# tudelft-iv/instance_stixels

Hardware: NVIDIA B200
Metric: stixel frames/sec @1024x2048 (higher is better)
Workload: dtype f32

## Files before the change

### instance_stixels_b200/csrc/context.cu

```cuda
#include <algorithm>
#include <cstdio>
#include <cstdlib>
#include <cstring>
#include <map>
#include <mutex>
#include <string>
#include <vector>

#include "host_model.h"
#include "kernels.h"

namespace isx {

static thread_local std::string g_last_error;
constexpr int kStageSlots = 8;
constexpr int kRoadSlots = 4;
constexpr int kResultSets = 4;
constexpr int kProfEvents = 9;
constexpr int kTraceStamps = 11;

static int fail(isx_context *ctx, int code, const std::string &msg);

struct RoadKey {
  int vhor;
  float tilt, height, alpha;
  bool operator<(const RoadKey &o) const {
    if (vhor != o.vhor) return vhor < o.vhor;
    if (tilt != o.tilt) return tilt < o.tilt;
    if (height != o.height) return height < o.height;
    return alpha < o.alpha;
  }
};

}

struct isx_context {
  int device = 0;
  bool configured_parts[8] = {false, false, false, false, false, false, false, false};
  bool initialized = false;
  isx::HostModel model;
  isx::KParams kp{};
  int max_batch = 0, chunk = 0;
  int chunk_unary = 0;
  int last_launch_frames = 0;
  std::string last_error;

  cudaStream_t s_tables = nullptr, s_compute = nullptr, s_emit = nullptr, s_h2d = nullptr, s_d2h = nullptr;
  cudaEvent_t ev_dp_done[2] = {nullptr, nullptr}, ev_emit_done[2] = {nullptr, nullptr};
  cudaEvent_t ev_tab_done[2] = {nullptr, nullptr};
  cudaEvent_t ev_user = nullptr;
  cudaEvent_t ev_in_ready[2] = {nullptr, nullptr}, ev_in_free[2] = {nullptr, nullptr};
  cudaEvent_t ev_chunk_done = nullptr;
  uint16_t *d_in_disp16[2] = {nullptr, nullptr};
  int16_t *d_in_seg16[2] = {nullptr, nullptr};

  std::vector<void *> allocations;
  float *d_in_disp[2] = {nullptr, nullptr};
  int32_t *d_in_seg[2] = {nullptr, nullptr};
  float *d_single_disp = nullptr;
  int32_t *d_single_seg = nullptr;
  isx::BatchBuffers buf;
  struct ChunkSet {
    float *stat = nullptr;
    uint32_t *records_b = nullptr;
    float4 *dp = nullptr;
    float *pm = nullptr;
    int *err = nullptr;
    float *joined = nullptr;
    float *object_lut = nullptr;
    int *col_flags = nullptr;
  } sets[2];
  int last_set = 0;
  struct RoadSlot {
    float *ground = nullptr;
    int *vhor = nullptr;
    cudaEvent_t ev_free = nullptr;
  } roads[isx::kRoadSlots];
  unsigned long long road_next = 0;
  int last_road_slot = 0;
  bool overlap_tables = true;
  bool emit_join_pending = false;
  struct ResultSet {
    bool allocated = false;
    isx_section *d_sections = nullptr;
    int *d_nsections = nullptr;
    isx_instance *d_inst = nullptr;
    int *d_inst_count = nullptr;
    int *d_cursors = nullptr;
    isx_section *h_sections = nullptr, *m_sections = nullptr;
    isx_instance *h_inst = nullptr, *m_inst = nullptr;
    int *h_counts = nullptr, *m_counts = nullptr;
    isx_packed_frame *h_frames = nullptr, *m_frames = nullptr;
    int sections_cap = 0, inst_cap = 0;
  } rs[isx::kResultSets];
  int cur = 0;
  int *d_raster_table = nullptr;
  int *d_export_col = nullptr;
  int inst_cap = 0;
  float *d_export_cost = nullptr;
  int *d_export_index = nullptr;

  float *h_ground = nullptr;
  int *h_vhor = nullptr;
  cudaEvent_t ev_stage_done[8] = {nullptr, nullptr, nullptr, nullptr, nullptr, nullptr, nullptr, nullptr};
  unsigned long long stage_next = 0;
  cudaEvent_t ev_batch_done[isx::kResultSets] = {};
  int batch_n[isx::kResultSets] = {};
  int batch_set[isx::kResultSets] = {};
  isx_section *batch_sections[isx::kResultSets] = {};
  bool batch_direct[isx::kResultSets] = {};
  isx_section *direct_sections = nullptr;
  bool results_stay_on_device = false;
  int last_waited_set = -1;
  unsigned long long submitted = 0, waited = 0;
  unsigned long long dp_units_pairwise = 0;
  unsigned long long dp_units_total = 0;
  int host_slot = 0;

  std::map<isx::RoadKey, std::vector<float>> road_cache;
  std::mutex road_cache_mutex;
  isx_road *h_stage_roads = nullptr;
  isx_road *d_batch_roads = nullptr;
  bool last_roads_device = false;
  isx_road single_road{0, 0.f, 0.f, 0.f};
  bool single_has_road = false;
  int last_batch = 0;
  int last_chunk_first = 0;
  int last_chunk_n = 0;
  bool last_pairwise = false;
  std::vector<isx_road> last_roads;
// ... 133 lines not shown
  ISX_TRY(c, cudaEventRecord(c->ev_stage_done[stage], st));
  return rslot;
}

static int stage_road_tables(isx_context *c, const isx_road *roads, int n, cudaStream_t st) {
  const int H = c->kp.rows;
  const int stage = (int)(c->stage_next++ % kStageSlots);
  ISX_TRY(c, cudaEventSynchronize(c->ev_stage_done[stage]));
  float *hg = c->h_ground + (size_t)stage * c->chunk * 3 * H;
  int *hv = c->h_vhor + (size_t)stage * c->chunk;
  for (int i = 0; i < n; i++) {
    copy_road_tables(c, roads[i], hg + (size_t)i * 3 * H);
    hv[i] = H - roads[i].vhor - 1;
  }
  return send_road_tables(c, stage, n, st);
}

struct StageFill {
  isx_context *c;
  int stage, n;
};

static void CUDART_CB fill_stage_from_roads(void *arg) {
  const StageFill p = *static_cast<StageFill *>(arg);
  delete static_cast<StageFill *>(arg);
  isx_context *c = p.c;
  const int H = c->kp.rows;
  const isx_road *roads = c->h_stage_roads + (size_t)p.stage * c->chunk;
  float *hg = c->h_ground + (size_t)p.stage * c->chunk * 3 * H;
  int *hv = c->h_vhor + (size_t)p.stage * c->chunk;
  for (int i = 0; i < p.n; i++) {
    copy_road_tables(c, roads[i], hg + (size_t)i * 3 * H);
    hv[i] = H - roads[i].vhor - 1;
  }
}

static int stage_device_road_tables(isx_context *c, const isx_road *d_roads, int n, cudaStream_t st) {
  const int stage = (int)(c->stage_next++ % kStageSlots);
  ISX_TRY(c, cudaStreamWaitEvent(st, c->ev_stage_done[stage], 0));
  ISX_TRY(c, cudaMemcpyAsync(c->h_stage_roads + (size_t)stage * c->chunk, d_roads, sizeof(isx_road) * n,
                             cudaMemcpyDeviceToHost, st));
  ISX_TRY(c, cudaLaunchHostFunc(st, fill_stage_from_roads, new StageFill{c, stage, n}));
  return send_road_tables(c, stage, n, st);
}

static int enqueue_chunk(isx_context *c, bool pairwise, int first, int n, const float *d_disp,
                         const int32_t *d_seg, const isx_road *roads, int slot, int road_slot = -1) {
  const KParams &kp = c->kp;
  const int H = kp.rows, C = kp.realcols;
  const isx_context::ChunkSet &cs = c->sets[slot];
  cudaStream_t st = c->s_tables, s = c->s_compute, se = c->s_emit;
  ISX_TRY(c, cudaStreamWaitEvent(st, c->ev_emit_done[slot], 0));
  if (!c->overlap_tables) ISX_TRY(c, cudaStreamWaitEvent(st, c->ev_dp_done[slot ^ 1], 0));
  if (road_slot < 0) {
    road_slot = stage_road_tables(c, roads, n, st);
    if (road_slot < 0) return road_slot;
  }
  const isx_context::RoadSlot &rd = c->roads[road_slot];
  ISX_TRY(c, cudaMemsetAsync(cs.err, 0, sizeof(int) * n, st));
  isx_context::ResultSet &R = c->rs[c->cur];
  BatchBuffers b = c->buf;
  b.ground = rd.ground; b.vhor = rd.vhor; b.stat = cs.stat;
  b.records_b = cs.records_b; b.dp = cs.dp; b.pm = cs.pm;
  b.joined = cs.joined; b.object_lut = cs.object_lut; b.col_flags = cs.col_flags;
  b.error_flag = cs.err;
  b.disparity = d_disp;
  b.segmentation = d_seg;
  b.sections = R.d_sections + (size_t)first * C * kMaxSections;
  b.n_sections = R.d_nsections + (size_t)first * C;
  auto mark = [&](cudaStream_t st) {
    if (!c->profiling) return;
    if (c->prof_used >= c->prof_events.size()) {
      cudaEvent_t e;
      cudaEventCreate(&e);
      c->prof_events.push_back(e);
    }
    cudaEventRecord(c->prof_events[c->prof_used++], st);
  };
  mark(st);
  launch_join_columns(kp, b, n, st);
  mark(st);
  if (pairwise) launch_frame_tables(kp, b, n, st);
  mark(st);
  launch_column_tables(kp, b, n, st);
  mark(st);
  ISX_TRY(c, cudaEventRecord(c->ev_tab_done[slot], st));
  ISX_TRY(c, cudaStreamWaitEvent(s, c->ev_tab_done[slot], 0));
  mark(s);
  launch_dp(kp, b, n, pairwise, s);
  {
    const unsigned long long nt = (unsigned long long)(H + 31) / 32;
    c->dp_units_total += (unsigned long long)n * C * (nt * (nt + 1) / 2);
    const char *ex = std::getenv("ISX_UNARY_EXHAUSTIVE");
    const bool walks_all = (pairwise && !pairwise_walk_used(n * C, b.qrows != nullptr)) || (!pairwise && ex && std::atoi(ex) != 0);
    c->dp_units_pairwise += walks_all ? (unsigned long long)n * C * (nt * (nt + 1) / 2) : 0;
  }
  mark(s);
  ISX_TRY(c, cudaEventRecord(c->ev_dp_done[slot], s));
  ISX_TRY(c, cudaStreamWaitEvent(se, c->ev_dp_done[slot], 0));
  mark(se);
  launch_emit(kp, b, n, pairwise, se);
  mark(se);
  launch_grouping(kp, b, n, se);
  {
    PackArgs a;
    a.sections = b.sections; a.n_sections = b.n_sections;
    a.cand_count = b.cand_count; a.cand_idx = b.cand_idx; a.cand_label = b.cand_label;
    a.err = cs.err; a.col_offset = b.pack_offset;
    a.inst_out = R.d_inst + (size_t)first * c->inst_cap; a.inst_count_out = R.d_inst_count + first;
    a.inst_cap = c->inst_cap; a.cursors = R.d_cursors;
    a.h_padded = c->direct_sections ? c->direct_sections + (size_t)first * C * kMaxSections : nullptr;
    a.h_sections = R.m_sections; a.h_sections_cap = c->results_stay_on_device ? 0 : R.sections_cap;
    a.h_inst = R.m_inst; a.h_inst_cap = c->results_stay_on_device ? 0 : R.inst_cap;
    a.h_counts = R.m_counts + (size_t)first * C; a.h_frames = R.m_frames + first;
    launch_pack(kp, a, n, se);
  }
  mark(se);
  ISX_TRY(c, cudaEventRecord(c->ev_emit_done[slot], se));
  ISX_TRY(c, cudaEventRecord(rd.ev_free, se));
  ISX_TRY(c, cudaGetLastError());
  c->last_chunk_first = first;
  c->last_chunk_n = n;
  c->last_pairwise = pairwise;
  c->last_set = slot;
  c->last_road_slot = road_slot;
  return ISX_OK;
}

static isx_section *device_view_of(isx_section *sections) {
  if (!sections) return nullptr;
  if (const char *e = std::getenv("ISX_NO_DIRECT"))
    if (std::atoi(e) != 0) return nullptr;
  cudaPointerAttributes attr;
  if (cudaPointerGetAttributes(&attr, sections) != cudaSuccess) {
    cudaGetLastError();
    return nullptr;
  }
  if (attr.type != cudaMemoryTypeHost || !attr.devicePointer) return nullptr;
  return static_cast<isx_section *>(attr.devicePointer);
}

static int begin_batch(isx_context *c) {
  ISX_TRY(c, cudaMemsetAsync(c->rs[c->cur].d_cursors, 0, 2 * sizeof(int), c->s_emit));
  return ISX_OK;
}

static int alloc_result_set(isx_context *c, int i) {
  isx_context::ResultSet &R = c->rs[i];
  if (R.allocated) return ISX_OK;
  const size_t C = c->kp.realcols, MB = c->max_batch;
  ISX_TRY(c, dev_alloc(c, &R.d_sections, MB * C * kMaxSections));
  ISX_TRY(c, cudaMemset(R.d_sections, 0, MB * C * kMaxSections * sizeof(isx_section)));
  ISX_TRY(c, dev_alloc(c, &R.d_nsections, MB * C));
  ISX_TRY(c, dev_alloc(c, &R.d_inst, MB * (size_t)c->inst_cap));
  ISX_TRY(c, dev_alloc(c, &R.d_inst_count, MB));
  ISX_TRY(c, dev_alloc(c, &R.d_cursors, 2));
  ISX_TRY(c, cudaMemset(R.d_cursors, 0, 2 * sizeof(int)));
  size_t budget = 100;
  if (c->kp.rows > kShortRows) budget = ((size_t)c->kp.rows * 100 + kShortRows - 1) / kShortRows;
  if (const char *e = std::getenv("ISX_PACK_BUDGET")) budget = std::atoi(e) > 0 ? (size_t)std::atoi(e) : budget;
  budget = budget < (size_t)kMaxSections ? budget : (size_t)kMaxSections;
  R.sections_cap = R.inst_cap = (int)(MB * C * budget);
  const unsigned flags = cudaHostAllocMapped | cudaHostAllocPortable;
  ISX_TRY(c, cudaHostAlloc(&R.h_sections, sizeof(isx_section) * (size_t)R.sections_cap, flags));
  ISX_TRY(c, cudaHostAlloc(&R.h_inst, sizeof(isx_instance) * (size_t)R.inst_cap, flags));
  ISX_TRY(c, cudaHostAlloc(&R.h_counts, sizeof(int) * MB * C, flags));
  ISX_TRY(c, cudaHostAlloc(&R.h_frames, sizeof(isx_packed_frame) * MB, flags));
// ... 108 lines not shown
  m.prior_weight = prior_weight; m.disparity_weight = disparity_weight; m.segmentation_weight = segmentation_weight;
  m.instance_weight = 0.0;
  if (segmentation_weight > 1e-5) {
    m.instance_weight = instance_weight / segmentation_weight;
    if (instance_weight < 1e-8) m.instance_weight = 0.0;
  }
  return ISX_OK;
}
int isx_set_probabilities(isx_handle h, float pout, float pout_sky, float pground_given_nexist,
                          float pobject_given_nexist, float psky_given_nexist, float pnexist_dis, float pground,
                          float pobject, float psky, float pord, float pgrav, float pblg) {
  if (!h) return fail(h, ISX_ERR_INVALID_ARGUMENT, "null handle");
  HostModel &m = h->model;
  m.pout = pout; m.pout_sky = pout_sky;
  m.pnexists_given_ground = (pground_given_nexist * pnexist_dis) / pground;
  m.pnexists_given_object = (pobject_given_nexist * pnexist_dis) / pobject;
  m.pnexists_given_sky = (psky_given_nexist * pnexist_dis) / psky;
  m.pord = pord; m.pgrav = pgrav; m.pblg = pblg;
  return ISX_OK;
}
int isx_set_camera_parameters(isx_handle h, float focal, float baseline, float sigma_camera_tilt,
                              float sigma_camera_height, float camera_center_x, float camera_center_y) {
  if (!h) return fail(h, ISX_ERR_INVALID_ARGUMENT, "null handle");
  HostModel &m = h->model;
  m.focal = focal; m.baseline = baseline;
  m.sigma_camera_tilt = sigma_camera_tilt * (3.1416f) / 180.0f;
  m.sigma_camera_height = sigma_camera_height;
  m.camera_center_x = camera_center_x; m.camera_center_y = camera_center_y;
  return ISX_OK;
}
int isx_set_model_parameters(isx_handle h, int column_step, int median_join, float epsilon, float range_objects_z,
                             int width_margin) {
  if (!h) return fail(h, ISX_ERR_INVALID_ARGUMENT, "null handle");
  HostModel &m = h->model;
  m.column_step = column_step; m.median_join = median_join != 0; m.epsilon = epsilon;
  m.range_objects_z = range_objects_z; m.width_margin = width_margin;
  return ISX_OK;
}

int isx_initialize(isx_handle h, int max_batch) {
  if (!h) return fail(h, ISX_ERR_INVALID_ARGUMENT, "null handle");
  if (h->initialized) return fail(h, ISX_ERR_INVALID_ARGUMENT, "already initialized: call Finish() first");
  if (max_batch < 1) return fail(h, ISX_ERR_INVALID_ARGUMENT, "max_batch must be >= 1");
  HostModel &m = h->model;
  if (m.rows <= 0 || m.cols <= 0 || m.max_dis <= 0 || m.column_step <= 0)
    return fail(h, ISX_ERR_INVALID_ARGUMENT, "configuration is not set");
  if (m.rows > ISX_MAX_ROWS) return fail(h, ISX_ERR_UNSUPPORTED, "rows > ISX_MAX_ROWS (2047) is not supported");
  if (m.max_dis > 256) return fail(h, ISX_ERR_UNSUPPORTED, "max_dis > 256 is not supported");
  if (m.n_classes != 19 || m.n_channels != 21)
    return fail(h, ISX_ERR_UNSUPPORTED, "the Cityscapes layout (19 classes + 2 offsets) is hard-wired like Cityscapes.h");
  if (m.column_step > 16) return fail(h, ISX_ERR_UNSUPPORTED, "column_step > 16 is not supported");
  ISX_TRY(h, cudaSetDevice(h->device));
  m.derive();
  fill_kparams(h);
  const KParams &kp = h->kp;
  const size_t H = kp.rows, W = kp.cols, C = kp.realcols, D = kp.max_dis;
  if (C == 0) return fail(h, ISX_ERR_INVALID_ARGUMENT, "no stixel columns");
  h->max_batch = max_batch;
  int chunk = 64, chunk_unary = 32;
  if (m.rows > kShortRows) {
    const size_t budget = 64 * chunk_frame_bytes(kShortRows, 2048, kRecStride, 2048 / 4, m.max_dis);
    const size_t per_frame = chunk_frame_bytes(m.rows, m.cols, rec_stride_for_rows(m.rows), m.realcols, m.max_dis);
    const size_t fit = budget / per_frame;
    chunk = fit < 1 ? 1 : fit < 64 ? (int)fit : 64;
    chunk_unary = chunk < 32 ? chunk : 32;
  }
  if (const char *e = std::getenv("ISX_CHUNK")) chunk = chunk_unary = std::atoi(e) > 0 ? std::atoi(e) : chunk;
  h->chunk = chunk < max_batch ? chunk : max_batch;
  h->chunk_unary = chunk_unary < h->chunk ? chunk_unary : h->chunk;
  h->last_launch_frames = h->chunk_unary;
  h->kp.lut_cols = h->chunk * (int)C;
  const size_t ch = h->chunk, MB = max_batch;
  const size_t cap = C * kMaxSections;
  h->inst_cap = (int)cap;

  {
    int prio_lo = 0, prio_hi = 0;
    ISX_TRY(h, cudaDeviceGetStreamPriorityRange(&prio_lo, &prio_hi));
    int prio_mid = prio_lo;
    if (const char *e = std::getenv("ISX_TABLES_PRIO"))
      prio_mid = (std::atoi(e) != 0 && prio_hi < prio_lo - 1) ? prio_hi + 1 : prio_lo;
    ISX_TRY(h, cudaStreamCreateWithPriority(&h->s_compute, cudaStreamNonBlocking, prio_lo));
    ISX_TRY(h, cudaStreamCreateWithPriority(&h->s_tables, cudaStreamNonBlocking, prio_mid));
    ISX_TRY(h, cudaStreamCreateWithPriority(&h->s_emit, cudaStreamNonBlocking, prio_hi));
  }
  ISX_TRY(h, cudaStreamCreateWithFlags(&h->s_h2d, cudaStreamNonBlocking));
  ISX_TRY(h, cudaStreamCreateWithFlags(&h->s_d2h, cudaStreamNonBlocking));
  for (int i = 0; i < 2; i++) {
    ISX_TRY(h, cudaEventCreateWithFlags(&h->ev_in_ready[i], cudaEventDisableTiming));
    ISX_TRY(h, cudaEventCreateWithFlags(&h->ev_in_free[i], cudaEventDisableTiming));
    ISX_TRY(h, cudaEventCreateWithFlags(&h->ev_dp_done[i], cudaEventDisableTiming));
    ISX_TRY(h, cudaEventCreateWithFlags(&h->ev_emit_done[i], cudaEventDisableTiming));
    ISX_TRY(h, cudaEventCreateWithFlags(&h->ev_tab_done[i], cudaEventDisableTiming));
  }
  ISX_TRY(h, cudaEventCreateWithFlags(&h->ev_chunk_done, cudaEventDisableTiming));
  ISX_TRY(h, cudaEventCreateWithFlags(&h->ev_user, cudaEventDisableTiming));

  BatchBuffers &b = h->buf;
  for (int i = 0; i < kRoadSlots; i++) {
    ISX_TRY(h, dev_alloc(h, &h->roads[i].ground, ch * 3 * H));
    ISX_TRY(h, dev_alloc(h, &h->roads[i].vhor, ch));
    ISX_TRY(h, cudaEventCreateWithFlags(&h->roads[i].ev_free, cudaEventDisableTiming));
  }
  h->road_next = 0;
  for (int i = 0; i < 2; i++) {
    ISX_TRY(h, dev_alloc(h, &h->d_in_disp[i], ch * H * W));
    ISX_TRY(h, dev_alloc(h, &h->d_in_seg[i], ch * seg_elems(h)));
    ISX_TRY(h, cudaMemset(h->d_in_seg[i], 0, ch * seg_elems(h) * sizeof(int32_t)));
  }
  ISX_TRY(h, dev_alloc(h, &h->d_single_disp, H * W));
  ISX_TRY(h, dev_alloc(h, &h->d_single_seg, seg_elems(h)));
  for (int i = 0; i < 2; i++) {
    isx_context::ChunkSet &cs = h->sets[i];
    ISX_TRY(h, dev_alloc(h, &cs.stat, ch * H * kStatWords));
    ISX_TRY(h, dev_alloc(h, &cs.records_b, ch * C * kRecBWords * (size_t)kp.rec_stride));
    ISX_TRY(h, cudaMemset(cs.records_b, 0, ch * C * kRecBWords * (size_t)kp.rec_stride * sizeof(uint32_t)));
    ISX_TRY(h, dev_alloc(h, &cs.pm, ch * C * H));
    ISX_TRY(h, cudaMemset(cs.pm, 0, ch * C * H * sizeof(float)));
    ISX_TRY(h, dev_alloc(h, &cs.dp, ch * C * H));
    ISX_TRY(h, dev_alloc(h, &cs.err, ch));
    ISX_TRY(h, dev_alloc(h, &cs.joined, ch * C * H));
    ISX_TRY(h, dev_alloc(h, &cs.object_lut, lut_buffer_bytes(ch * C, D * (size_t)kp.lut_stride * 4) / 4));
    ISX_TRY(h, dev_alloc(h, &cs.col_flags, ch * C));
    ISX_TRY(h, cudaMemset(cs.col_flags, 0, ch * C * sizeof(int)));
  }
  ISX_TRY(h, dev_alloc(h, &b.cand_count, ch * kInstanceClasses));
  ISX_TRY(h, dev_alloc(h, &b.cand_offset, ch * (C + 1) * kInstanceClasses));
  ISX_TRY(h, dev_alloc(h, &b.cand_xy, ch * kInstanceClasses * cap));
  ISX_TRY(h, dev_alloc(h, &b.cand_idx, ch * kInstanceClasses * cap));
  ISX_TRY(h, dev_alloc(h, &b.cand_core, ch * kInstanceClasses * cap));
  ISX_TRY(h, dev_alloc(h, &b.cand_label, ch * kInstanceClasses * cap));
  ISX_TRY(h, dev_alloc(h, &b.cand_scratch, ch * kInstanceClasses * cap));
  ISX_TRY(h, dev_alloc(h, &b.pack_offset, ch * (C + 1)));
  ISX_TRY(h, dev_alloc(h, &b.dp_units, 1));
  if (pairwise_walk_enabled()) {
    ISX_TRY(h, dev_alloc(h, &b.qrows, ch * C * (size_t)kp.rec_stride * kDynWords));
    ISX_TRY(h, cudaMemset(b.qrows, 0, ch * C * (size_t)kp.rec_stride * kDynWords * sizeof(float)));
  }
  ISX_TRY(h, cudaMemset(b.dp_units, 0, sizeof(unsigned long long)));
  h->cur = 0;
  if (int rc = alloc_result_set(h, 0)) return rc;
  ISX_TRY(h, dev_alloc(h, &h->d_raster_table, MB * C * kMaxSections));
  ISX_TRY(h, dev_alloc(h, &h->d_export_col, MB * C));
  ISX_TRY(h, dev_alloc(h, &h->d_export_cost, C * H * 3));
  ISX_TRY(h, dev_alloc(h, &h->d_export_index, C * H * 3));

  float *d_tmp = nullptr;
  ISX_TRY(h, dev_alloc(h, &d_tmp, D * D));
  ISX_TRY(h, cudaMemcpy(d_tmp, m.obj_cost_lut.data(), sizeof(float) * D * D, cudaMemcpyHostToDevice));
  b.obj_cost_lut = d_tmp;
  {
    const size_t Dp = (D + 31) & ~(size_t)31;
    std::vector<float> t(D * Dp, 0.0f);
    for (size_t fn = 0; fn < D; fn++)
      for (size_t dis = 0; dis < D; dis++) t[dis * Dp + fn] = m.obj_cost_lut[fn * D + dis];
    ISX_TRY(h, dev_alloc(h, &d_tmp, 2 * D * Dp));
    const unsigned long long a0 = (unsigned long long)d_tmp, bytes = sizeof(float) * D * Dp;
    if (((a0 ^ (a0 + bytes - 1)) >> 32) != 0) d_tmp += D * Dp;
    ISX_TRY(h, cudaMemcpy(d_tmp, t.data(), bytes, cudaMemcpyHostToDevice));
    b.obj_cost_lut_t = d_tmp;
  }
  ISX_TRY(h, dev_alloc(h, &d_tmp, D));
  ISX_TRY(h, cudaMemcpy(d_tmp, m.object_disparity_range.data(), sizeof(float) * D, cudaMemcpyHostToDevice));
  b.object_disparity_range = d_tmp;
  ISX_TRY(h, dev_alloc(h, &d_tmp, H + 1));
  ISX_TRY(h, cudaMemcpy(d_tmp, m.inverse_height.data(), sizeof(float) * (H + 1), cudaMemcpyHostToDevice));
  b.inverse_height = d_tmp;

  ISX_TRY(h, cudaMallocHost(&h->h_ground, sizeof(float) * kStageSlots * ch * 3 * H));
  ISX_TRY(h, cudaMallocHost(&h->h_vhor, sizeof(int) * kStageSlots * ch));
  ISX_TRY(h, cudaMallocHost(&h->h_stage_roads, sizeof(isx_road) * kStageSlots * ch));
  ISX_TRY(h, dev_alloc(h, &h->d_batch_roads, MB));
  for (int i = 0; i < kStageSlots; i++) ISX_TRY(h, cudaEventCreateWithFlags(&h->ev_stage_done[i], cudaEventDisableTiming));
  h->stage_next = 0;
  h->road_cache.clear();
  h->overlap_tables = true;
  if (const char *e = std::getenv("ISX_OVERLAP_TABLES")) h->overlap_tables = std::atoi(e) != 0;
  h->initialized = true;
  h->last_batch = 0;
  return ISX_OK;
}

int isx_finish(isx_handle h) {
  if (!h) return fail(h, ISX_ERR_INVALID_ARGUMENT, "null handle");
  if (!h->initialized) return ISX_OK;
  cudaSetDevice(h->device);
  cudaDeviceSynchronize();
  for (void *p : h->allocations) cudaFree(p);
  h->allocations.clear();
  cudaFreeHost(h->h_ground);
  cudaFreeHost(h->h_vhor);
  cudaFreeHost(h->h_stage_roads);
  h->h_stage_roads = nullptr;
  h->d_batch_roads = nullptr;
  h->last_roads_device = false;
  for (int i = 0; i < kStageSlots; i++) {
    if (h->ev_stage_done[i]) cudaEventDestroy(h->ev_stage_done[i]);
    h->ev_stage_done[i] = nullptr;
  }
  for (int i = 0; i < kRoadSlots; i++) {
    if (h->roads[i].ev_free) cudaEventDestroy(h->roads[i].ev_free);
    h->roads[i] = isx_context::RoadSlot();
  }
  for (int i = 0; i < kResultSets; i++) {
    isx_context::ResultSet &R = h->rs[i];
    if (R.allocated) {
      cudaFreeHost(R.h_sections);
      cudaFreeHost(R.h_inst);
      cudaFreeHost(R.h_counts);
      cudaFreeHost(R.h_frames);
    }
    R = isx_context::ResultSet();
    if (h->ev_batch_done[i]) cudaEventDestroy(h->ev_batch_done[i]);
    h->ev_batch_done[i] = nullptr;
    h->batch_sections[i] = nullptr;
    h->batch_n[i] = 0;
  }
  for (int i = 0; i < 2; i++) {
    h->d_in_disp16[i] = nullptr;
    h->d_in_seg16[i] = nullptr;
  }
  h->cur = 0;
  h->submitted = h->waited = 0;
  h->last_waited_set = -1;
  h->host_slot = 0;
  h->dp_units_total = h->dp_units_pairwise = 0;
  h->emit_join_pending = false;
  for (int i = 0; i < 2; i++) {
    cudaEventDestroy(h->ev_in_ready[i]);
    cudaEventDestroy(h->ev_in_free[i]);
    cudaEventDestroy(h->ev_dp_done[i]);
    cudaEventDestroy(h->ev_emit_done[i]);
    cudaEventDestroy(h->ev_tab_done[i]);
  }
  cudaEventDestroy(h->ev_chunk_done);
  cudaEventDestroy(h->ev_user);
  cudaStreamDestroy(h->s_tables);
  cudaStreamDestroy(h->s_compute);
  cudaStreamDestroy(h->s_emit);
  cudaStreamDestroy(h->s_h2d);
  cudaStreamDestroy(h->s_d2h);
  h->buf = BatchBuffers();
  h->initialized = false;
  return ISX_OK;
}

int isx_is_initialized(isx_handle h) { return h && h->initialized; }
int isx_real_cols(isx_handle h) { return h ? (h->initialized ? h->kp.realcols : 0) : 0; }
int isx_max_sections(isx_handle h) { (void)h; return kMaxSections; }
size_t isx_segmentation_elems(isx_handle h) { return (h && h->initialized) ? seg_elems(h) : 0; }

int isx_set_disparity_image(isx_handle h, const float *host, size_t n) {
  if (int rc = check_ready(h)) return rc;
  if (!host || n != (size_t)h->kp.rows * h->kp.cols)
    return fail(h, ISX_ERR_INVALID_ARGUMENT, "disparity image must hold rows*cols floats");
  ISX_TRY(h, cudaMemcpyAsync(h->d_single_disp, host, n * sizeof(float), cudaMemcpyHostToDevice, h->s_tables));
  return ISX_OK;
}

float *isx_input_disparity_device(isx_handle h) {
  if (!h || !h->initialized) return nullptr;
  cudaSetDevice(h->device);
  cudaStreamSynchronize(h->s_tables);
  return h->d_single_disp;
}

int isx_set_segmentation(isx_handle h, const int32_t *host, size_t n) {
  if (int rc = check_ready(h)) return rc;
  if (!host || n != seg_elems(h))
    return fail(h, ISX_ERR_INVALID_ARGUMENT, "segmentation must hold realcols*channels*rows_power2_segmentation ints");
  ISX_TRY(h, cudaMemcpyAsync(h->d_single_seg, host, n * sizeof(int32_t), cudaMemcpyHostToDevice, h->s_tables));
  return ISX_OK;
}

static int check_cnn_grid(isx_handle h, int cnn_rows, int cnn_cols) {
  const KParams &kp = h->kp;
  if (kp.width_margin != 0 || kp.column_step < 1 || kDownsample % kp.column_step != 0)
    return fail(h, ISX_ERR_UNSUPPORTED, "segmentation ingest needs width_margin == 0 and column_step dividing 8");
  if (cnn_rows != kp.rows / kDownsample || cnn_cols * (kDownsample / kp.column_step) != kp.realcols)
    return fail(h, ISX_ERR_INVALID_ARGUMENT, "CNN output must be [channels][rows/8][cols/8]");
  return ISX_OK;
}

int isx_set_segmentation_from_cnn_device(isx_handle h, const float *d_cnn, int cnn_rows, int cnn_cols) {
  if (int rc = check_ready(h)) return rc;
  if (!d_cnn) return fail(h, ISX_ERR_INVALID_ARGUMENT, "null argument");
  if (int rc = check_cnn_grid(h, cnn_rows, cnn_cols)) return rc;
  launch_flip_and_pad(h->kp, d_cnn, h->d_single_seg, 1, cnn_rows, cnn_cols, h->s_tables);
  ISX_TRY(h, cudaGetLastError());
  return ISX_OK;
}

int isx_flip_and_pad_batch_device(isx_handle h, int n, const float *d_cnn, int cnn_rows, int cnn_cols,
                                  int32_t *d_segmentation) {
  if (int rc = check_ready(h)) return rc;
  if (!d_cnn || !d_segmentation || n < 1) return fail(h, ISX_ERR_INVALID_ARGUMENT, "null argument or empty batch");
  if (int rc = check_cnn_grid(h, cnn_rows, cnn_cols)) return rc;
  launch_flip_and_pad(h->kp, d_cnn, d_segmentation, n, cnn_rows, cnn_cols, h->s_tables);
  ISX_TRY(h, cudaGetLastError());
  return ISX_OK;
}

int isx_set_road_parameters(isx_handle h, int vhor, float camera_tilt, float camera_height, float alpha_ground) {
  if (!h) return fail(h, ISX_ERR_INVALID_ARGUMENT, "null handle");
  h->single_road = isx_road{vhor, camera_tilt, camera_height, alpha_ground};
  h->single_has_road = true;
  return ISX_OK;
}

static int no_batches_in_flight(isx_handle h);

static int deliver(isx_handle h, isx_context::ResultSet &R, int n, isx_section *sections, isx_instance *instances,
                   int instances_capacity, int32_t *instance_offsets, bool direct = false) {
  if (direct) sections = nullptr;
  const size_t C = h->kp.realcols;
  int rc = ISX_OK;
  int total = 0;
  for (int f = 0; f < n; f++) {
    const isx_packed_frame &d = R.h_frames[f];
    if (d.error && rc == ISX_OK) {
// ... 645 lines not shown
```

### instance_stixels_b200/csrc/kernels.h

```cpp
#pragma once
#include <cuda_runtime.h>
#include <stdint.h>

#include <atomic>
#include <string>

#include "../../include/instance_stixels_b200.h"
#include "common.cuh"

namespace isx {

struct BatchBuffers {
  const float *disparity = nullptr;
  const int32_t *segmentation = nullptr;
  float *ground = nullptr;
  int *vhor = nullptr;
  float *stat = nullptr;
  float *joined = nullptr;
  uint32_t *records_b = nullptr;
  float *object_lut = nullptr;
  float *pm = nullptr;
  float *qrows = nullptr;
  float4 *dp = nullptr;
  const float *obj_cost_lut = nullptr;
  const float *obj_cost_lut_t = nullptr;
  const float *object_disparity_range = nullptr;
  const float *inverse_height = nullptr;
  isx_section *sections = nullptr;
  int *n_sections = nullptr;
  int *cand_count = nullptr;
  int *cand_offset = nullptr;
  float2 *cand_xy = nullptr;
  int2 *cand_idx = nullptr;
  uint8_t *cand_core = nullptr;
  int *cand_label = nullptr;
  int *cand_scratch = nullptr;
  int *error_flag = nullptr;
  int *pack_offset = nullptr;
  int *col_flags = nullptr;
  unsigned long long *dp_units = nullptr;
};

void launch_join_columns(const KParams &p, const BatchBuffers &b, int nframes, cudaStream_t s);
void launch_frame_tables(const KParams &p, const BatchBuffers &b, int nframes, cudaStream_t s);
void launch_column_tables(const KParams &p, const BatchBuffers &b, int nframes, cudaStream_t s);
void launch_dp(const KParams &p, const BatchBuffers &b, int nframes, bool pairwise, cudaStream_t s);
bool pairwise_walk_enabled();
bool pairwise_walk_used(int ncolumns, bool have_qrows);
void launch_emit(const KParams &p, const BatchBuffers &b, int nframes, bool pairwise, cudaStream_t s);
void launch_flip_and_pad(const KParams &p, const float *cnn, int32_t *seg, int nframes, int hs, int ws,
                         cudaStream_t s);
void launch_rasterize(const KParams &p, const isx_section *sections, const int *n_sections, const isx_instance *inst,
                      const int *inst_count, int inst_cap, int *table, int nframes, uint8_t *label_img,
                      int32_t *instance_img, float *disparity_img, cudaStream_t s);
void launch_grouping(const KParams &p, const BatchBuffers &b, int nframes, cudaStream_t s);
struct PackArgs {
  const isx_section *sections;
  const int *n_sections;
  const int *cand_count;
  const int2 *cand_idx;
  const int *cand_label;
  const int *err;
  int *col_offset;
  isx_instance *inst_out;
  int *inst_count_out;
  int inst_cap;
  int *cursors;
  isx_section *h_sections;
  int h_sections_cap;
  isx_instance *h_inst;
  int h_inst_cap;
  isx_section *h_padded;
  int *h_counts;
  isx_packed_frame *h_frames;
};
void launch_pack(const KParams &p, const PackArgs &a, int nframes, cudaStream_t s);
struct ExportArgs {
  const isx_section *sections;
  const int *n_sections;
  const isx_instance *inst;
  const int *inst_count;
  int inst_cap;
  const isx_packed_frame *frames;
  int *col_local;
  int realcols, rows, column_step;
  float focal, bf, camera_center_x, camera_center_y;
  const isx_road *roads;
  isx_device_results out;
};
constexpr int kExportFramesPerLaunch = 128;
struct ExportFrames {
  float alpha_ground[kExportFramesPerLaunch];
  int vhor[kExportFramesPerLaunch];
};
void launch_export_results(const ExportArgs &a, int nframes, const float *alpha_ground, const int *vhor,
                           cudaStream_t s);
int road_check_batch(isx_road_handle road, int device, int rows, int cols, int max_dis, int n, bool has_fallback,
                     std::string &msg);
int road_enqueue_batch(isx_road_handle road, cudaStream_t caller, int n, const float *d_disparity,
                       const isx_road *fallback, isx_road_estimate *d_estimates, isx_road *d_roads_out,
                       isx_road *d_roads, std::string &msg);
void launch_widen_inputs(const KParams &p, const uint16_t *disp16, float scale, const int16_t *seg16, float *disp,
                         int32_t *seg, int nframes, cudaStream_t s);
int dbscan_fit_host(const float *xy, int n, float eps, int min_pts, const uint8_t *core_candidates, int *labels,
                    int threads);
void launch_export_tables(const KParams &p, const BatchBuffers &b, int frame, bool pairwise, float *cost_table,
                          int *index_table, cudaStream_t s);

extern std::atomic<unsigned long long> g_launch_count;

constexpr int kMaxDevices = 64;
inline int current_device() {
  int d = 0;
  cudaGetDevice(&d);
  return (d < 0 || d >= kMaxDevices) ? 0 : d;
}
inline int device_sm_count() {
  static std::atomic<int> sms[kMaxDevices];
  const int d = current_device();
  int n = sms[d].load(std::memory_order_relaxed);
  if (n == 0) {
    cudaDeviceGetAttribute(&n, cudaDevAttrMultiProcessorCount, d);
    sms[d].store(n, std::memory_order_relaxed);
  }
  return n;
}
struct SmemOptIn {
  std::atomic<int> done[kMaxDevices];
// ... 18 lines not shown
```

### instance_stixels_b200/csrc/tables.cu

```cuda
#include <cstdlib>
#include "kernels.h"

namespace isx {

namespace {

__global__ void frame_tables_kernel(const float *__restrict__ ground, const int *__restrict__ vhor_arr,
                                    float *__restrict__ stat, KParams p) {
  const int f = blockIdx.y;
  const int vB = blockIdx.x * blockDim.x + threadIdx.x;
  const int H = p.rows;
  if (vB >= H) return;
  float *S = stat + ((size_t)f * H + vB) * kStatWords;
  if (vB == 0) {
    for (int i = 0; i < kStatWords; i++) S[i] = 0.0f;
    return;
  }
  const float *gf = ground + (size_t)f * 3 * H;
  const int vhor = vhor_arr[f];
  const int pv = vB - 1;
  const float eps = p.epsilon;

  const float pc = ffma(lg2_approx((float)(H - vB)), kLn2, -0.0f);
  const float fnp = clamp_neg(gf[pv]);
// ... 24 lines not shown
    float x = v < H ? e[v] : 0.0f;
#pragma unroll
    for (int b = 0; b < 5; b++) x = fadd(x, __shfl_xor_sync(full, x, 1 << b));
    if constexpr (TALL) {
      if (lane == (k & 31)) {
        if (k < 32) total_k = x;
        else total2_k = x;
      }
    } else {
      if (lane == k) total_k = x;
    }
  }
  float y = total_k, left[5];
#pragma unroll
  for (int b = 0; b < 5; b++) {
    const float o = __shfl_xor_sync(full, y, 1 << b);
    left[b] = o;
    y = fadd(y, o);
  }
  float hi = 0.0f;
#pragma unroll
  for (int b = 4; b >= 0; b--)
    if ((lane >> b) & 1) hi = fadd(hi, left[b]);
  float hi2 = 0.0f;
  if constexpr (TALL) {
    float y2 = total2_k, left2[5];
#pragma unroll
    for (int b = 0; b < 5; b++) {
      const float o = __shfl_xor_sync(full, y2, 1 << b);
      left2[b] = o;
      y2 = fadd(y2, o);
    }
    hi2 = fadd(0.0f, y);
#pragma unroll
    for (int b = 4; b >= 0; b--)
      if ((lane >> b) & 1) hi2 = fadd(hi2, left2[b]);
  }
  const int kmax = H >> 5;
  for (int k = 0; k <= kmax; k++) {
    const int v = (k << 5) + lane;
    float x = v < H ? e[v] : 0.0f;
    float lo[5];
#pragma unroll
    for (int b = 0; b < 5; b++) {
      const float o = __shfl_xor_sync(full, x, 1 << b);
      lo[b] = o;
      x = fadd(x, o);
    }
    float pre;
    if constexpr (TALL) {
      pre = __shfl_sync(full, k < 32 ? hi : hi2, k & 31);
    } else {
      pre = (k < 32) ? __shfl_sync(full, hi, k & 31) : y;
    }
#pragma unroll
    for (int b = 4; b >= 0; b--)
      if ((lane >> b) & 1) pre = fadd(pre, lo[b]);
    if (v <= H) ps[v] = pre;
  }
}

template <typename T>
__device__ void exact_prefix_warp(const T *e, int n, T *ps) {
  const unsigned full = 0xffffffffu;
  const int lane = threadIdx.x & 31;
  T carry = 0;
  for (int base = 0; base < n; base += 32) {
    const int i = base + lane;
    T x = i < n ? e[i] : (T)0;
    T incl = x;
#pragma unroll
    for (int d = 1; d < 32; d <<= 1) {
      const T o = __shfl_up_sync(full, incl, d);
      if (lane >= d) incl += o;
    }
    if (i < n) ps[i] = carry + incl - x;
    carry += __shfl_sync(full, incl, 31);
  }
  if (lane == 0) ps[n] = carry;
}

constexpr int kTabThreads = 256;

struct TabSmem {
  int Hp, nq;
  size_t off_e[4], off_seg, off_i64, off_i32, total;
  __host__ __device__ TabSmem(int H, int hs2) {
    Hp = (H + 1 + 3) & ~3;
    nq = H / 8 + 1;
    size_t o = 0;
    off_i64 = o; o += (size_t)Hp * 8 * 2;
    off_i32 = o; o += (size_t)Hp * 4 * 2;
    for (int i = 0; i < 4; i++) { off_e[i] = o; o += (size_t)Hp * 4; }
    off_seg = o; o += (size_t)20 * (nq + 1) * 4;
    total = (o + 15) & ~(size_t)15;
    (void)hs2;
  }
};

template <bool TALL> struct TabLimits {
  static constexpr int kMeanRowLimit = TALL ? 1 << 19 : 1 << 20;
  static constexpr int kClassLimit = TALL ? 1 << 19 : 1 << 20;
  static constexpr int kSqOffLimit = TALL ? 1 << 18 : 1 << 19;
};

template <bool TALL>
__global__ void __launch_bounds__(kTabThreads, 4)
column_tables_kernel(const float *__restrict__ joined, const int32_t *__restrict__ segmentation,
                     const float *__restrict__ ground, const int *__restrict__ vhor_arr,
                     uint32_t *__restrict__ records_b, int *__restrict__ error_flag, int *__restrict__ col_flags,
                     KParams p) {
  extern __shared__ __align__(16) unsigned char smem[];
  const int H = p.rows, C = p.realcols;
  const int col = blockIdx.x, f = blockIdx.y;
  const int tid = threadIdx.x, warp = tid >> 5, lane = tid & 31;
  const TabSmem L(H, p.hs2);
  float *e_disp = reinterpret_cast<float *>(smem + L.off_e[0]);
  float *e_valid = reinterpret_cast<float *>(smem + L.off_e[1]);
  float *e_ground = reinterpret_cast<float *>(smem + L.off_e[2]);
  float *e_sky = reinterpret_cast<float *>(smem + L.off_e[3]);
  long long *ps_i64 = reinterpret_cast<long long *>(smem + L.off_i64);
  int *ps_i32 = reinterpret_cast<int *>(smem + L.off_i32);
  int *seg_ps = reinterpret_cast<int *>(smem + L.off_seg);
  const int nq = L.nq, segld = nq + 1;

  const float *d_col = joined + ((size_t)f * C + col) * H;
  const int32_t *seg_col = segmentation + ((size_t)f * C + col) * p.n_channels * p.hs2;
  const float *gf = ground + (size_t)f * 3 * H;
  const float *norm_g = gf + H, *inv_g = gf + 2 * H;
  const int vhor = vhor_arr[f];
  const float invalid = p.invalid_disparity;
  const int K = p.n_classes;
  const bool has_oy = K < p.n_channels, has_ox = K + 1 < p.n_channels;
  constexpr int kMeanRowLimit = TabLimits<TALL>::kMeanRowLimit;

  bool negative_class_value = false;
#pragma unroll
  for (int c = warp; c < 20; c += kTabThreads / 32) {
#pragma unroll 5
    for (int q = lane; q < nq; q += 32) {
      int v = 0;
      if (c < K) {
        if (c < p.n_channels && q < p.hs2) v = __ldg(seg_col + (size_t)c * p.hs2 + q);
        negative_class_value |= v < 0 || v > TabLimits<TALL>::kClassLimit;
      } else {
        int oy = 0, ox = 0;
        if (q < p.hs2 && has_oy) oy = __ldg(seg_col + (size_t)K * p.hs2 + q);
        if (q < p.hs2 && has_ox) ox = __ldg(seg_col + (size_t)(K + 1) * p.hs2 + q);
        oy = oy * oy;
        ox = ox * ox;
        negative_class_value |= oy < 0 || oy > TabLimits<TALL>::kSqOffLimit || ox < 0 ||
                                ox > TabLimits<TALL>::kSqOffLimit;
        v = oy + ox;
      }
      seg_ps[c * segld + q] = v;
    }
  }
  bool out_of_range = false;
  for (int v0 = tid; v0 < H; v0 += 4 * kTabThreads) {
    float d4[4], g0[4], gi[4], gn[4];
    int oy4[4], ox4[4];
#pragma unroll
    for (int j = 0; j < 4; j++) {
      const int v = v0 + j * kTabThreads;
      const bool ok = v < H;
      const int q = v / kDownsample;
      d4[j] = ok ? __ldg(d_col + v) : 0.0f;
      oy4[j] = (ok && q < p.hs2 && has_oy) ? __ldg(seg_col + (size_t)K * p.hs2 + q) : 0;
      ox4[j] = (ok && q < p.hs2 && has_ox) ? __ldg(seg_col + (size_t)(K + 1) * p.hs2 + q) : 0;
      const bool gr = ok && v < vhor;
      g0[j] = gr ? __ldg(gf + v) : 0.0f;
      gi[j] = gr ? __ldg(inv_g + v) : 0.0f;
      gn[j] = gr ? __ldg(norm_g + v) : 0.0f;
    }
#pragma unroll
    for (int j = 0; j < 4; j++) {
      const int v = v0 + j * kTabThreads;
      if (v >= H) break;
      const float d = d4[j];
      if (invalid >= 0.0f) {
        const int va = d != invalid;
        e_valid[v] = (float)va;
        e_disp[v] = fmul((float)va, d);
      } else {
        e_valid[v] = 1.0f;
        e_disp[v] = d;
      }
      float sky = 0.0f;
      if (v >= vhor) {
        sky = p.pnexists_given_sky_log;
        if (d != invalid) {
          const float g = ffma(fmul(d, d), p.inv_sigma2_sky, p.normalization_sky);
          sky = fadd(fmin_(g, p.puniform_sky), p.nopnexists_given_sky_log);
        }
      }
      e_sky[v] = sky;
      float grd = inf_f();
      if (v < vhor) {
        grd = p.pnexists_given_ground_log;
        if (d != invalid) {
          const float diff = fsub(d, g0[j]);
          const float g = ffma(fmul(diff, diff), gi[j], gn[j]);
          grd = fadd(fmin_(g, p.puniform), p.nopnexists_given_ground_log);
        }
      }
      e_ground[v] = grd;
      const long long mx = (long long)((p.column_step * col + 0.5 * (p.column_step - 1.0)) + ox4[j] + 0.5);
      const long long my = (long long)(v - oy4[j] + 0.5);
      out_of_range |= mx <= -kMeanRowLimit || mx >= kMeanRowLimit || my <= -kMeanRowLimit || my >= kMeanRowLimit;
      ps_i32[0 * L.Hp + v] = (int)mx;
      ps_i32[1 * L.Hp + v] = (int)my;
      ps_i64[0 * L.Hp + v] = mx * mx;
      ps_i64[1 * L.Hp + v] = my * my;
    }
  }
  const int any_negative = __syncthreads_or(negative_class_value ? 1 : 0);
  if (tid == 0) col_flags[(size_t)f * C + col] = any_negative;

  if (warp < 4) {
    blelloch_prefix_warp<TALL>(e_disp + warp * L.Hp, H, e_disp + warp * L.Hp);
  } else if (warp < 6) {
    exact_prefix_warp<long long>(ps_i64 + (warp - 4) * L.Hp, H, ps_i64 + (warp - 4) * L.Hp);
  } else {
    exact_prefix_warp<int>(ps_i32 + (warp - 6) * L.Hp, H, ps_i32 + (warp - 6) * L.Hp);
  }
  for (int c = 19 - ((warp + 4) & 7); c >= 0; c -= kTabThreads / 32)
    exact_prefix_warp<int>(seg_ps + c * segld, nq, seg_ps + c * segld);
  __syncthreads();

  uint4 *recb_col = reinterpret_cast<uint4 *>(records_b + ((size_t)f * C + col) * (size_t)p.rec_stride * kRecBWords);
  const long long lim2 = 1ll << (24 + kSqSplitBits);
  const int lim1 = 1 << 24;
  const long long lomask = (1ll << kSqSplitBits) - 1;
  const int g = tid & 7, r = (tid >> 3) & 7;
  const int *ps_grp = seg_ps + (4 * (g < 5 ? g : 4)) * segld;
  const long long *ps_sq = ps_i64 + (g == 5 ? 0 : L.Hp);
  const float *pf_a = g == 6 ? e_disp : e_ground, *pf_b = g == 6 ? e_valid : e_sky;
#pragma unroll 2
  for (int v = tid >> 3; v <= H; v += kTabThreads / 8) {
    uint4 w;
    {
      const int *ps = ps_grp + (v >> 3);
      const int a0 = ps[0], a1 = ps[segld], a2 = ps[2 * segld], a3 = ps[3 * segld];
      w.x = (uint32_t)(a0 * kDownsample + (ps[1] - a0) * r);
      w.y = (uint32_t)(a1 * kDownsample + (ps[segld + 1] - a1) * r);
      w.z = (uint32_t)(a2 * kDownsample + (ps[2 * segld + 1] - a2) * r);
      w.w = (uint32_t)(a3 * kDownsample + (ps[3 * segld + 1] - a3) * r);
    }
    if (g >= 5) {
      const int smx = ps_i32[0 * L.Hp + v], smy = ps_i32[1 * L.Hp + v];
      const long long sq = ps_sq[v];
      out_of_range |= (g == 5 && (smx <= -lim1 || smx >= lim1 || smy <= -lim1 || smy >= lim1)) || (g != 7 && sq >= lim2);
      const float hi = (float)(sq & ~lomask), lo = (float)(sq & lomask);
      const float fa = pf_a[v], fb = pf_b[v];
      w.x = __float_as_uint(g == 5 ? (float)smx : g == 6 ? hi : fa);
      w.y = __float_as_uint(g == 5 ? (float)smy : g == 6 ? lo : fb);
      w.z = g == 7 ? 0u : __float_as_uint(g == 5 ? hi : fa);
      w.w = g == 7 ? 0u : __float_as_uint(g == 5 ? lo : fb);
    }
    recb_col[v * (kRecBWords / 4) + g] = w;
  }
  if (out_of_range) atomicOr(error_flag + f, kErrOffsetRange);
}

constexpr int kLutWarps = 4;
constexpr int kLutThreads = kLutWarps * 32;

__device__ __forceinline__ float ldg_lo_hi(unsigned lo, unsigned hi) {
  float r;
  asm("{\n\t.reg .b64 a;\n\tmov.b64 a, {%1, %2};\n\tld.global.nc.f32 %0, [a];\n\t}" : "=f"(r) : "r"(lo), "r"(hi));
  return r;
}
__device__ __forceinline__ void stg_lo_hi(unsigned lo, unsigned hi, float v) {
  asm volatile("{\n\t.reg .b64 a;\n\tmov.b64 a, {%0, %1};\n\tst.global.f32 [a], %2;\n\t}" ::"r"(lo), "r"(hi), "f"(v)
               : "memory");
}

template <int MAXH>
__global__ void __launch_bounds__(kLutThreads)
object_lut_kernel(const float *__restrict__ joined, const float *__restrict__ cost_t,
                  float *__restrict__ object_lut, KParams p) {
  __shared__ __align__(16) uint8_t dis_s[MAXH + 32];
  __shared__ float tile[kLutWarps][32][33];
  const int H = p.rows, C = p.realcols, D = p.max_dis;
  const int Dp = (D + 31) & ~31;
  const int col = blockIdx.x, f = blockIdx.z;
  const int warp = threadIdx.x >> 5, lane = threadIdx.x & 31;
  const float *d_col = joined + ((size_t)f * C + col) * H;
  const int Hc = (H + 31) & ~31;
  for (int v = threadIdx.x; v < Hc; v += kLutThreads) {
    int di = 0;
    if (v < H) {
      di = (int)d_col[v];
      di = di < 0 ? 0 : (di >= D ? D - 1 : di);
    }
    dis_s[v] = (uint8_t)di;
  }
  __syncthreads();
  const int fn0 = (blockIdx.y * kLutWarps + warp) * 32;
  if (fn0 >= D) return;
  const unsigned long long lut_addr = lut_column_address((unsigned long long)object_lut, (size_t)f * C + col,
                                                         p.lut_cols, (size_t)D * p.lut_stride * 4);
  const unsigned lut_hi = (unsigned)(lut_addr >> 32);
  const unsigned stride4 = (unsigned)p.lut_stride * 4u;
  const unsigned long long cost_addr = (unsigned long long)(cost_t + fn0 + lane);
  const unsigned cost_lo = (unsigned)cost_addr, cost_hi = (unsigned)(cost_addr >> 32);
  const unsigned row4 = (unsigned)Dp * 4u;
  float(*tl)[33] = tile[warp];
  const bool full = fn0 + 32 <= D;
  float carry = 0.0f;
  for (int i = 0; i < Hc; i += 32) {
    float x[32];
    const uint4 *dq = reinterpret_cast<const uint4 *>(dis_s + i);
    const uint4 d0 = dq[0], d1 = dq[1];
    const uint32_t dw[8] = {d0.x, d0.y, d0.z, d0.w, d1.x, d1.y, d1.z, d1.w};
#pragma unroll
    for (int r = 0; r < 32; r++) {
      const unsigned dis = __byte_perm(dw[r >> 2], 0u, 0x4440u | (unsigned)(r & 3));
      x[r] = ldg_lo_hi(dis * row4 + cost_lo, cost_hi);
    }
    x[0] = fadd(x[0], carry);
#pragma unroll
    for (int j = 1; j < 32; j <<= 1) {
#pragma unroll
      for (int L = 31; L >= j; L--) x[L] = fadd(x[L], x[L - j]);
    }
    carry = x[31];
    __syncwarp();
#pragma unroll
    for (int r = 0; r < 32; r++) tl[lane][r] = x[r];
    __syncwarp();
    const int v = i + lane;
    if (v < H) {
      unsigned lo = (unsigned)lut_addr + (unsigned)fn0 * stride4 + 4u * (unsigned)v;
      if (full) {
#pragma unroll
        for (int r = 0; r < 32; r++) {
          stg_lo_hi(lo, lut_hi, tl[r][lane]);
          lo += stride4;
        }
      } else {
#pragma unroll
        for (int r = 0; r < 32; r++) {
          if (fn0 + r < D) stg_lo_hi(lo, lut_hi, tl[r][lane]);
          lo += stride4;
        }
      }
    }
  }
}

}

void launch_frame_tables(const KParams &p, const BatchBuffers &b, int nframes, cudaStream_t s) {
  dim3 grid((p.rows + 255) / 256, nframes);
  frame_tables_kernel<<<grid, 256, 0, s>>>(b.ground, b.vhor, b.stat, p);
  g_launch_count++;
}

static size_t tab_smem_bytes(const KParams &p) { return TabSmem(p.rows, p.hs2).total; }

static size_t padded_smem(size_t need, size_t static_bytes) {
  static const int n = [] {
    const char *e = std::getenv("ISX_TAB_CTAS_PER_SM");
    return e ? std::atoi(e) : 0;
  }();
  if (n <= 0) return need;
  const size_t per_cta = (size_t)(227 * 1024) / (size_t)(n + 1) + 1024;
  const size_t want = per_cta > static_bytes + 1024 ? per_cta - static_bytes - 1024 : 0;
  return want > need ? want : need;
}

template <bool TALL>
static void launch_column_tables_rows(const KParams &p, const BatchBuffers &b, int nframes, cudaStream_t s) {
  constexpr int kLutMaxH = TALL ? 2048 : 1024;
  dim3 grid(p.realcols, nframes);
  const size_t smem = padded_smem(tab_smem_bytes(p), 0);
  static SmemOptIn optin, optin_lut;
  opt_in_smem(column_tables_kernel<TALL>, optin);
  opt_in_smem(object_lut_kernel<kLutMaxH>, optin_lut);
  column_tables_kernel<TALL><<<grid, kTabThreads, smem, s>>>(b.joined, b.segmentation, b.ground, b.vhor, b.records_b,
                                                              b.error_flag, b.col_flags, p);
  dim3 lgrid(p.realcols, (p.max_dis + 32 * kLutWarps - 1) / (32 * kLutWarps), nframes);
  object_lut_kernel<kLutMaxH><<<lgrid, kLutThreads, padded_smem(0, sizeof(float) * kLutWarps * 32 * 33 + kLutMaxH + 32), s>>>(
      b.joined, b.obj_cost_lut_t, b.object_lut, p);
  g_launch_count += 2;
}

void launch_column_tables(const KParams &p, const BatchBuffers &b, int nframes, cudaStream_t s) {
  if (p.rows > kShortRows) launch_column_tables_rows<true>(p, b, nframes, s);
  else launch_column_tables_rows<false>(p, b, nframes, s);
}

}
```

Baseline: 8232.

## Run object LUT concurrently on side stream and stage record writes through shared memory

Moves the object LUT kernel onto a new stream forked from the tables stream, so it can overlap with the column tables kernel and join back before the DP. Also restructures the record-B write loop in column_tables_kernel: each warp produces one record slot for 32 rows into a swizzled shared-memory block, then threads write full contiguous rows to global memory to coalesce stores. This adds shared memory per CTA and two block barriers per 32-row step, which may reduce occupancy.

```diff
diff --git a/instance_stixels_b200/csrc/context.cu b/instance_stixels_b200/csrc/context.cu
--- a/instance_stixels_b200/csrc/context.cu
+++ b/instance_stixels_b200/csrc/context.cu
@@ -46,6 +46,8 @@
   std::string last_error;
 
   cudaStream_t s_tables = nullptr, s_compute = nullptr, s_emit = nullptr, s_h2d = nullptr, s_d2h = nullptr;
+  cudaStream_t s_lut = nullptr;
+  cudaEvent_t ev_lut_fork = nullptr, ev_lut_done = nullptr;
   cudaEvent_t ev_dp_done[2] = {nullptr, nullptr}, ev_emit_done[2] = {nullptr, nullptr};
   cudaEvent_t ev_tab_done[2] = {nullptr, nullptr};
   cudaEvent_t ev_user = nullptr;
@@ -345,7 +347,12 @@
   mark(st);
   if (pairwise) launch_frame_tables(kp, b, n, st);
   mark(st);
+  ISX_TRY(c, cudaEventRecord(c->ev_lut_fork, st));
+  ISX_TRY(c, cudaStreamWaitEvent(c->s_lut, c->ev_lut_fork, 0));
   launch_column_tables(kp, b, n, st);
+  launch_object_lut(kp, b, n, c->s_lut);
+  ISX_TRY(c, cudaEventRecord(c->ev_lut_done, c->s_lut));
+  ISX_TRY(c, cudaStreamWaitEvent(st, c->ev_lut_done, 0));
   mark(st);
   ISX_TRY(c, cudaEventRecord(c->ev_tab_done[slot], st));
   ISX_TRY(c, cudaStreamWaitEvent(s, c->ev_tab_done[slot], 0));
@@ -620,6 +627,7 @@
       prio_mid = (std::atoi(e) != 0 && prio_hi < prio_lo - 1) ? prio_hi + 1 : prio_lo;
     ISX_TRY(h, cudaStreamCreateWithPriority(&h->s_compute, cudaStreamNonBlocking, prio_lo));
     ISX_TRY(h, cudaStreamCreateWithPriority(&h->s_tables, cudaStreamNonBlocking, prio_mid));
+    ISX_TRY(h, cudaStreamCreateWithPriority(&h->s_lut, cudaStreamNonBlocking, prio_mid));
     ISX_TRY(h, cudaStreamCreateWithPriority(&h->s_emit, cudaStreamNonBlocking, prio_hi));
   }
   ISX_TRY(h, cudaStreamCreateWithFlags(&h->s_h2d, cudaStreamNonBlocking));
@@ -632,6 +640,8 @@
     ISX_TRY(h, cudaEventCreateWithFlags(&h->ev_tab_done[i], cudaEventDisableTiming));
   }
   ISX_TRY(h, cudaEventCreateWithFlags(&h->ev_chunk_done, cudaEventDisableTiming));
+  ISX_TRY(h, cudaEventCreateWithFlags(&h->ev_lut_fork, cudaEventDisableTiming));
+  ISX_TRY(h, cudaEventCreateWithFlags(&h->ev_lut_done, cudaEventDisableTiming));
   ISX_TRY(h, cudaEventCreateWithFlags(&h->ev_user, cudaEventDisableTiming));
 
   BatchBuffers &b = h->buf;
@@ -772,8 +782,11 @@
     cudaEventDestroy(h->ev_tab_done[i]);
   }
   cudaEventDestroy(h->ev_chunk_done);
+  cudaEventDestroy(h->ev_lut_fork);
+  cudaEventDestroy(h->ev_lut_done);
   cudaEventDestroy(h->ev_user);
   cudaStreamDestroy(h->s_tables);
+  cudaStreamDestroy(h->s_lut);
   cudaStreamDestroy(h->s_compute);
   cudaStreamDestroy(h->s_emit);
   cudaStreamDestroy(h->s_h2d);
diff --git a/instance_stixels_b200/csrc/kernels.h b/instance_stixels_b200/csrc/kernels.h
--- a/instance_stixels_b200/csrc/kernels.h
+++ b/instance_stixels_b200/csrc/kernels.h
@@ -44,6 +44,7 @@
 void launch_join_columns(const KParams &p, const BatchBuffers &b, int nframes, cudaStream_t s);
 void launch_frame_tables(const KParams &p, const BatchBuffers &b, int nframes, cudaStream_t s);
 void launch_column_tables(const KParams &p, const BatchBuffers &b, int nframes, cudaStream_t s);
+void launch_object_lut(const KParams &p, const BatchBuffers &b, int nframes, cudaStream_t s);
 void launch_dp(const KParams &p, const BatchBuffers &b, int nframes, bool pairwise, cudaStream_t s);
 bool pairwise_walk_enabled();
 bool pairwise_walk_used(int ncolumns, bool have_qrows);
diff --git a/instance_stixels_b200/csrc/tables.cu b/instance_stixels_b200/csrc/tables.cu
--- a/instance_stixels_b200/csrc/tables.cu
+++ b/instance_stixels_b200/csrc/tables.cu
@@ -130,13 +130,17 @@
 
 constexpr int kTabThreads = 256;
 
+constexpr int kRecBlockRows = 32;
+static_assert(kRecBlockRows * (kRecBWords / 4) == kTabThreads, "one 16-byte slot of the block per thread");
+
 struct TabSmem {
   int Hp, nq;
-  size_t off_e[4], off_seg, off_i64, off_i32, total;
+  size_t off_rec, off_e[4], off_seg, off_i64, off_i32, total;
   __host__ __device__ TabSmem(int H, int hs2) {
     Hp = (H + 1 + 3) & ~3;
     nq = H / 8 + 1;
     size_t o = 0;
+    off_rec = o; o += (size_t)kRecBlockRows * kRecBWords * 4;
     off_i64 = o; o += (size_t)Hp * 8 * 2;
     off_i32 = o; o += (size_t)Hp * 4 * 2;
     for (int i = 0; i < 4; i++) { off_e[i] = o; o += (size_t)Hp * 4; }
@@ -277,36 +281,45 @@
   __syncthreads();
 
   uint4 *recb_col = reinterpret_cast<uint4 *>(records_b + ((size_t)f * C + col) * (size_t)p.rec_stride * kRecBWords);
+  uint4 *rec_blk = reinterpret_cast<uint4 *>(smem + L.off_rec);
   const long long lim2 = 1ll << (24 + kSqSplitBits);
   const int lim1 = 1 << 24;
   const long long lomask = (1ll << kSqSplitBits) - 1;
-  const int g = tid & 7, r = (tid >> 3) & 7;
-  const int *ps_grp = seg_ps + (4 * (g < 5 ? g : 4)) * segld;
-  const long long *ps_sq = ps_i64 + (g == 5 ? 0 : L.Hp);
-  const float *pf_a = g == 6 ? e_disp : e_ground, *pf_b = g == 6 ? e_valid : e_sky;
-#pragma unroll 2
-  for (int v = tid >> 3; v <= H; v += kTabThreads / 8) {
-    uint4 w;
-    {
-      const int *ps = ps_grp + (v >> 3);
-      const int a0 = ps[0], a1 = ps[segld], a2 = ps[2 * segld], a3 = ps[3 * segld];
-      w.x = (uint32_t)(a0 * kDownsample + (ps[1] - a0) * r);
-      w.y = (uint32_t)(a1 * kDownsample + (ps[segld + 1] - a1) * r);
-      w.z = (uint32_t)(a2 * kDownsample + (ps[2 * segld + 1] - a2) * r);
-      w.w = (uint32_t)(a3 * kDownsample + (ps[3 * segld + 1] - a3) * r);
-    }
-    if (g >= 5) {
-      const int smx = ps_i32[0 * L.Hp + v], smy = ps_i32[1 * L.Hp + v];
-      const long long sq = ps_sq[v];
-      out_of_range |= (g == 5 && (smx <= -lim1 || smx >= lim1 || smy <= -lim1 || smy >= lim1)) || (g != 7 && sq >= lim2);
-      const float hi = (float)(sq & ~lomask), lo = (float)(sq & lomask);
-      const float fa = pf_a[v], fb = pf_b[v];
-      w.x = __float_as_uint(g == 5 ? (float)smx : g == 6 ? hi : fa);
-      w.y = __float_as_uint(g == 5 ? (float)smy : g == 6 ? lo : fb);
-      w.z = g == 7 ? 0u : __float_as_uint(g == 5 ? hi : fa);
-      w.w = g == 7 ? 0u : __float_as_uint(g == 5 ? lo : fb);
-    }
-    recb_col[v * (kRecBWords / 4) + g] = w;
+  const int r = lane & 7;
+  const int *ps_grp = seg_ps + 4 * (warp < 5 ? warp : 0) * segld;
+  const int srow = tid >> 3, sslot = (tid & 7) ^ (srow & 7);
+  for (int v0 = 0; v0 <= H; v0 += kRecBlockRows) {
+    const int v = v0 + lane;
+    if (v <= H) {
+      uint4 w;
+      if (warp < 5) {
+        const int *ps = ps_grp + (v >> 3);
+        const int a0 = ps[0], a1 = ps[segld], a2 = ps[2 * segld], a3 = ps[3 * segld];
+        w.x = (uint32_t)(a0 * kDownsample + (ps[1] - a0) * r);
+        w.y = (uint32_t)(a1 * kDownsample + (ps[segld + 1] - a1) * r);
+        w.z = (uint32_t)(a2 * kDownsample + (ps[2 * segld + 1] - a2) * r);
+        w.w = (uint32_t)(a3 * kDownsample + (ps[3 * segld + 1] - a3) * r);
+      } else if (warp < 7) {
+        const long long sq = ps_i64[(warp - 5) * L.Hp + v];
+        out_of_range |= sq >= lim2;
+        const float hi = (float)(sq & ~lomask), lo = (float)(sq & lomask);
+        if (warp == 5) {
+          const int smx = ps_i32[0 * L.Hp + v], smy = ps_i32[1 * L.Hp + v];
+          out_of_range |= smx <= -lim1 || smx >= lim1 || smy <= -lim1 || smy >= lim1;
+          w = make_uint4(__float_as_uint((float)smx), __float_as_uint((float)smy), __float_as_uint(hi),
+                         __float_as_uint(lo));
+        } else {
+          w = make_uint4(__float_as_uint(hi), __float_as_uint(lo), __float_as_uint(e_disp[v]),
+                         __float_as_uint(e_valid[v]));
+        }
+      } else {
+        w = make_uint4(__float_as_uint(e_ground[v]), __float_as_uint(e_sky[v]), 0u, 0u);
+      }
+      rec_blk[lane * 8 + (warp ^ r)] = w;
+    }
+    __syncthreads();
+    if (v0 + srow <= H) recb_col[(v0 + srow) * (kRecBWords / 4) + (tid & 7)] = rec_blk[srow * 8 + sslot];
+    __syncthreads();
   }
   if (out_of_range) atomicOr(error_flag + f, kErrOffsetRange);
 }
@@ -421,18 +434,13 @@
 
 template <bool TALL>
 static void launch_column_tables_rows(const KParams &p, const BatchBuffers &b, int nframes, cudaStream_t s) {
-  constexpr int kLutMaxH = TALL ? 2048 : 1024;
   dim3 grid(p.realcols, nframes);
   const size_t smem = padded_smem(tab_smem_bytes(p), 0);
-  static SmemOptIn optin, optin_lut;
+  static SmemOptIn optin;
   opt_in_smem(column_tables_kernel<TALL>, optin);
-  opt_in_smem(object_lut_kernel<kLutMaxH>, optin_lut);
   column_tables_kernel<TALL><<<grid, kTabThreads, smem, s>>>(b.joined, b.segmentation, b.ground, b.vhor, b.records_b,
                                                               b.error_flag, b.col_flags, p);
-  dim3 lgrid(p.realcols, (p.max_dis + 32 * kLutWarps - 1) / (32 * kLutWarps), nframes);
-  object_lut_kernel<kLutMaxH><<<lgrid, kLutThreads, padded_smem(0, sizeof(float) * kLutWarps * 32 * 33 + kLutMaxH + 32), s>>>(
-      b.joined, b.obj_cost_lut_t, b.object_lut, p);
-  g_launch_count += 2;
+  g_launch_count++;
 }
 
 void launch_column_tables(const KParams &p, const BatchBuffers &b, int nframes, cudaStream_t s) {
@@ -440,4 +448,19 @@
   else launch_column_tables_rows<false>(p, b, nframes, s);
 }
 
-}
+template <int MAXH>
+static void launch_object_lut_rows(const KParams &p, const BatchBuffers &b, int nframes, cudaStream_t s) {
+  static SmemOptIn optin;
+  opt_in_smem(object_lut_kernel<MAXH>, optin);
+  dim3 grid(p.realcols, (p.max_dis + 32 * kLutWarps - 1) / (32 * kLutWarps), nframes);
+  object_lut_kernel<MAXH><<<grid, kLutThreads, padded_smem(0, sizeof(float) * kLutWarps * 32 * 33 + MAXH + 32), s>>>(
+      b.joined, b.obj_cost_lut_t, b.object_lut, p);
+  g_launch_count++;
+}
+
+void launch_object_lut(const KParams &p, const BatchBuffers &b, int nframes, cudaStream_t s) {
+  if (p.rows > kShortRows) launch_object_lut_rows<2048>(p, b, nframes, s);
+  else launch_object_lut_rows<1024>(p, b, nframes, s);
+}
+
+}
```

Result: faster. 8494, median of 6 (+3.2%).
